# RishWijewardhena/vision-textile-inspection

Hardware: AMD Instinct MI355X
Metric: frames/sec whole-node, YOLOv8n-seg 640x640 bs=64; mask IoU vs CPU ref (higher is better)
Workload: dtype f16x2

## Files before the change

### vision-textile-inspection_amd/csrc/post.hip

```cpp
#include <algorithm>
#include <cmath>
#include <cstdio>
#include <cstring>
#include <type_traits>
#include <vector>

#include "vti_internal.h"

namespace vti {

typedef _Float16 half_t;
typedef _Float16 half8 __attribute__((ext_vector_type(8)));
typedef float f32x4 __attribute__((ext_vector_type(4)));

struct LinTap { int s0, s1, a0, a1; };

__device__ __forceinline__ LinTap lin_tap(int d, int ssize, double scale, bool horizontal) {
    float f = (float)(((double)d + 0.5) * scale - 0.5);
    int s = (int)floorf(f);
    f -= (float)s;
    LinTap t;
    if (horizontal) {
        if (s < 0) { s = 0; f = 0.f; }
        if (s >= ssize - 1) { s = ssize - 1; f = 0.f; }
// ... 217 lines not shown
                if (i >= (nc >> 2)) continue;
                if (v[u].x > best) { best = v[u].x; j = 4 * i; }
                if (v[u].y > best) { best = v[u].y; j = 4 * i + 1; }
                if (v[u].z > best) { best = v[u].z; j = 4 * i + 2; }
                if (v[u].w > best) { best = v[u].w; j = 4 * i + 3; }
            }
            for (int i = q + 4 * MAXV; i < (nc >> 2); i += 4) {
                const float4 w = row[i];
                if (w.x > best) { best = w.x; j = 4 * i; }
                if (w.y > best) { best = w.y; j = 4 * i + 1; }
                if (w.z > best) { best = w.z; j = 4 * i + 2; }
                if (w.w > best) { best = w.w; j = 4 * i + 3; }
            }
        }
#pragma unroll
        for (int o = 1; o <= 2; o <<= 1) {
            const float ob = __shfl_xor(best, o);
            const int oj = __shfl_xor(j, o);
            if (ob > best || (ob == best && oj < j)) { best = ob; j = oj; }
        }
        if (q != 0 || a >= A) return;
    } else {
        a = blockIdx.x * 256 + threadIdx.x;
        if (a >= A) return;
        const float* P = pred + ((size_t)b * A + a) * no;
        best = P[4];
        for (int c = 1; c < nc; ++c) {
            const float v = P[4 + c];
            if (v > best) { best = v; j = c; }
        }
    }
    if (best_out) {
        *(float2*)(best_out + ((size_t)b * A + a) * 2) = make_float2(best, (float)(j == 0x7fffffff ? 0 : j));
        return;
    }
    if (best > conf) {
        char* wsb = ws + (size_t)b * L.per_frame;
        const int idx = atomicAdd(&ncand[b], 1);
        ((unsigned long long*)(wsb + L.keys))[idx] = ((unsigned long long)(~__float_as_uint(best)) << 32) | (unsigned)a;
        ((int*)(wsb + L.cls))[a] = j;
    }
}

#ifdef VTI_STAMPS
__device__ unsigned long long g_nms_stamps[4096 * 8];
#define NMS_STAMP(i)                                                                                   \
    do {                                                                                               \
        if (tid == 0 && b < 4096) {                                                                    \
            unsigned long long t_;                                                                     \
            asm volatile("s_memtime %0\n\ts_waitcnt lgkmcnt(0)" : "=s"(t_)::"memory");                 \
            g_nms_stamps[b * 8 + (i)] = t_;                                                            \
        }                                                                                              \
    } while (0)
#else
#define NMS_STAMP(i) do { } while (0)
#endif

template <typename KeyP, typename BoxP, typename FltP, typename IntP>
__device__ __forceinline__ void nms_body(const float* __restrict__ P, int A, int nc, int nm, int n, double iou, int max_det,
                                         int agnostic, float* __restrict__ D, int* __restrict__ counts, int b,
                                         const unsigned long long* __restrict__ g_keys_in, KeyP keys, BoxP boxes, FltP area,
                                         IntP keep, IntP kid, IntP kcls, unsigned char* suppressed,
                                         const int* __restrict__ cls_of) {
    const int tid = threadIdx.x;
    int Pn = 1;
    while (Pn < n) Pn <<= 1;
    for (int i = tid; i < Pn; i += NMS_THREADS) keys[i] = i < n ? g_keys_in[i] : ~0ull;
    __syncthreads();
    for (int k = 2; k <= Pn; k <<= 1) {
        for (int j = k >> 1; j > 0; j >>= 1) {
            for (int i = tid; i < Pn; i += NMS_THREADS) {
                const int ixj = i ^ j;
                if (ixj > i) {
                    const unsigned long long x = keys[i], y = keys[ixj];
                    const bool up = (i & k) == 0;
                    if ((x > y) == up) { keys[i] = y; keys[ixj] = x; }
                }
            }
            __syncthreads();
        }
    }
    NMS_STAMP(1);
    if (n > NMS_MAX_NMS) n = NMS_MAX_NMS;
    for (int i = tid; i < n; i += NMS_THREADS) {
        const int a = (int)(keys[i] & 0xffffffffu);
        const float* Pa = P + (size_t)a * (4 + nc + nm);
        const float cx = Pa[0], cy = Pa[1], w = Pa[2], h = Pa[3];
        const float dw = w / 2.0f, dh = h / 2.0f;
        const float off = agnostic ? 0.0f : (float)cls_of[a] * NMS_MAX_WH;
        f32x4 bx;
        bx[0] = (cx - dw) + off; bx[1] = (cy - dh) + off; bx[2] = (cx + dw) + off; bx[3] = (cy + dh) + off;
        boxes[i] = bx;
        area[i] = (bx[2] - bx[0]) * (bx[3] - bx[1]);
        suppressed[i] = 0;
    }
    __syncthreads();
    NMS_STAMP(2);
    __shared__ unsigned long long s_rows[64];
    __shared__ int s_kept;
    auto iou_gt = [&](const f32x4& bi, float ai, const f32x4& bj, float aj) -> bool {
        const float xx1 = fmaxf(bi[0], bj[0]), yy1 = fmaxf(bi[1], bj[1]);
        const float xx2 = fminf(bi[2], bj[2]), yy2 = fminf(bi[3], bj[3]);
        const float w = fmaxf(0.0f, xx2 - xx1), h = fmaxf(0.0f, yy2 - yy1);
        const float inter = w * h;
        const float ovr = inter / (ai + aj - inter);
        return (double)ovr > iou;
    };
    int kept = 0;
    if (tid == 0) s_kept = 0;
    for (int base = 0; base < n && kept < max_det; base += 64) {
        const int cnt = min(64, n - base);
        if (tid < 64) s_rows[tid] = 0;
        __syncthreads();
        for (int e = tid; e < 64 * 16; e += NMS_THREADS) {
            const int i = e >> 4, jg = (e & 15) * 4;
            if (i >= cnt || jg + 3 <= i) continue;
            const f32x4 bi = boxes[base + i];
            const float ai = area[base + i];
            unsigned long long m = 0;
            f32x4 bj4[4];
            float aj4[4];
#pragma unroll
            for (int k = 0; k < 4; ++k) {
                const int jc = jg + k < cnt ? jg + k : cnt - 1;
                bj4[k] = boxes[base + jc]; aj4[k] = area[base + jc];
            }
#pragma unroll
            for (int k = 0; k < 4; ++k) {
                const int j = jg + k;
                if (j > i && j < cnt && iou_gt(bi, ai, bj4[k], aj4[k])) m |= 1ull << j;
            }
            if (m) atomicOr(&s_rows[i], m);
        }
        __syncthreads();
        if (tid < 64) {
            const bool alive_l = tid < cnt && !suppressed[base + tid];
            unsigned long long alive = __ballot(alive_l);
            int k_ = kept;
            const unsigned long long myrow = s_rows[tid];
            const int row_lo = (int)(unsigned)myrow, row_hi = (int)(unsigned)(myrow >> 32);
            while (alive && k_ < max_det) {
                const int i = __ffsll((long long)alive) - 1;
                if (tid == 0) keep[k_] = base + i;
                ++k_;
                const unsigned long long ri = (unsigned long long)(unsigned)__builtin_amdgcn_readlane(row_lo, i) |
                                              ((unsigned long long)(unsigned)__builtin_amdgcn_readlane(row_hi, i) << 32);
                alive &= ~(ri | (1ull << i));
            }
            if (tid == 0) s_kept = k_;
        }
        __syncthreads();
        const int kept0 = kept;
        kept = s_kept;
        if (kept < max_det) {
            const int nk = kept - kept0;
            const int rest = n - (base + 64);
            int parts = 1;
            while (parts < 8 && rest * parts * 2 <= NMS_THREADS) parts <<= 1;
            const int part = tid & (parts - 1), lane_j = tid / parts, jstep = NMS_THREADS / parts;
            for (int j = base + 64 + lane_j; j < n; j += jstep) {
                if (suppressed[j]) continue;
                const f32x4 bj = boxes[j];
                const float aj = area[j];
                bool sup = false;
                for (int t = 4 * part; t < nk && !sup; t += 4 * parts) {
                    int ii[4];
                    f32x4 bk[4];
                    float ak[4];
#pragma unroll
                    for (int u = 0; u < 4; ++u) ii[u] = keep[kept0 + (t + u < nk ? t + u : nk - 1)];
#pragma unroll
                    for (int u = 0; u < 4; ++u) { bk[u] = boxes[ii[u]]; ak[u] = area[ii[u]]; }
#pragma unroll
                    for (int u = 0; u < 4; ++u) sup = sup | iou_gt(bk[u], ak[u], bj, aj);
                }
                if (sup) suppressed[j] = 1;
            }
        }
        __syncthreads();
    }
    NMS_STAMP(3);
    for (int k = tid; k < kept; k += NMS_THREADS) {
        const int a = (int)(keys[keep[k]] & 0xffffffffu);
        kid[k] = a;
        kcls[k] = cls_of[a];
    }
    __syncthreads();
    const int row = 6 + nm;
    const unsigned row_magic = (unsigned)((0x100000000ull + (unsigned)row - 1) / (unsigned)row);
    const int nel = kept * row, ntot = max_det * row;
    const int no_ = 4 + nc + nm;
    constexpr int OU = 8;
    for (int e0 = tid; e0 < nel; e0 += OU * NMS_THREADS) {
        float x1[OU], x2[OU];
        int fj[OU];
#pragma unroll
        for (int u = 0; u < OU; ++u) {
            const int e = e0 + u * NMS_THREADS;
            const int ec = e < nel ? e : 0;
            const int k = (int)__umulhi((unsigned)ec, row_magic), f = ec - k * row;
            const int a = kid[k], j = kcls[k];
            const int off1 = f < 4 ? (f & 1) : f == 4 ? 4 + j : f == 5 ? 0 : 4 + nc + (f - 6);
            const int off2 = f < 4 ? 2 + (f & 1) : off1;
            const float* Pa = P + (size_t)a * no_;
            x1[u] = Pa[off1]; x2[u] = Pa[off2];
            fj[u] = (f << 16) | j;
        }
#pragma unroll
        for (int u = 0; u < OU; ++u) {
            const int e = e0 + u * NMS_THREADS;
            const int f = fj[u] >> 16, j = fj[u] & 0xffff;
            const float d_ = x2[u] / 2.0f;
            const float v = f < 2 ? x1[u] - d_ : f < 4 ? x1[u] + d_ : f == 5 ? (float)j : x1[u];
            if (e < nel) D[e] = v;
        }
    }
    for (int e = nel + tid; e < ntot; e += NMS_THREADS) D[e] = 0.f;
    __syncthreads();
    NMS_STAMP(4);
    if (tid == 0) counts[b] = kept;
}

__global__ __launch_bounds__(NMS_THREADS) void nms_kernel(const float* __restrict__ pred, int A, int nc, int nm,
                                                          float conf, double iou, int max_det, int agnostic,
                                                          float* __restrict__ dets, int* __restrict__ counts,
                                                          char* ws, NmsWsLayout L, int* __restrict__ ncand,
                                                          const float* __restrict__ best) {
    extern __shared__ __attribute__((aligned(16))) char smem[];
    unsigned long long* lds_keys = (unsigned long long*)smem;
    f32x4* lds_boxes = (f32x4*)(smem + NMS_LDS_KEYS * 8);
    float* lds_area = (float*)(lds_boxes + NMS_LDS_BOX);
    int* lds_keep = (int*)(lds_area + NMS_LDS_BOX);
    unsigned char* suppressed = (unsigned char*)(lds_keep + 3 * NMS_LDS_BOX);

// ... 39 lines not shown
                 lds_keep + NMS_LDS_BOX, lds_keep + 2 * NMS_LDS_BOX, suppressed, cls_of);
    } else {
        int* g_int = (int*)(wsb + L.keep);
        nms_body(P, A, nc, nm, n, iou, max_det, agnostic, D, counts, b, g_keys, (unsigned long long*)(wsb + L.keys2),
                 (f32x4*)(wsb + L.boxes), (float*)(wsb + L.area), g_int, (int*)(wsb + L.kid), (int*)(wsb + L.kcls), suppressed,
                 cls_of);
    }
}

hipError_t launch_anchor_best(const float* pred, int B, int A, int nc, int nm, float* best, hipStream_t st) {
    if (B == 0) return hipSuccess;
    const int apb = (((4 + nc + nm) | nc) & 3) == 0 ? 64 : 256;
    hipLaunchKernelGGL(nms_scan_kernel, dim3((A + apb - 1) / apb, B), dim3(256), 0, st, pred, A, nc, nm, 0.0f, (char*)nullptr, nms_layout(A),
                       (int*)nullptr, best);
    return hipGetLastError();
}

hipError_t launch_nms(const float* pred, const float* best, int B, int A, int nc, int nm, float conf, double iou, int max_det,
                      int agnostic, float* dets, int* counts, void* ws, hipStream_t st) {
    if (B == 0) return hipSuccess;
    const size_t lds = (size_t)NMS_LDS_KEYS * 8 + (size_t)NMS_LDS_BOX * 32 + (((size_t)A + 15) & ~(size_t)15);
    if (lds > 150 * 1024) return hipErrorInvalidValue;
    const NmsWsLayout L = nms_layout(A);
    int* ncand = (int*)((char*)ws + L.per_frame * (size_t)B);
    if (!best) {
        hipError_t e = hipMemsetAsync(ncand, 0, sizeof(int) * (size_t)B, st);
        if (e != hipSuccess) return e;
        const int apb = (((4 + nc + nm) | nc) & 3) == 0 ? 64 : 256;
        hipLaunchKernelGGL(nms_scan_kernel, dim3((A + apb - 1) / apb, B), dim3(256), 0, st, pred, A, nc, nm, conf, (char*)ws, L, ncand, (float*)nullptr);
    }
    const hipError_t e = launch_lds<nms_kernel>(dim3(B), dim3(NMS_THREADS), lds, st, pred, A, nc, nm, conf, iou, max_det, agnostic,
                                                dets, counts, (char*)ws, L, ncand, best);
#ifdef VTI_STAMPS
    {
        (void)hipStreamSynchronize(st);
        static int calls = 0;
        if (++calls == 3) {
            std::vector<unsigned long long> h(4096 * 8);
            std::vector<int> hc(B), hn(B);
            (void)hipMemcpyFromSymbol(h.data(), HIP_SYMBOL(g_nms_stamps), h.size() * 8);
            (void)hipMemcpy(hc.data(), counts, B * 4, hipMemcpyDeviceToHost);
            (void)hipMemcpy(hn.data(), ncand, B * 4, hipMemcpyDeviceToHost);
            const char* nm_[4] = {"sort", "boxes", "greedy", "output"};
            int worst = 0;
            for (int b = 1; b < B; ++b) if (h[b * 8 + 4] - h[b * 8] > h[worst * 8 + 4] - h[worst * 8]) worst = b;
            fprintf(stderr, "[nms stamps] slowest frame %d: candidates %d kept %d\n", worst, hn[worst], hc[worst]);
            for (int i = 0; i < 4; ++i) {
                std::vector<long long> d;
                for (int b = 0; b < B; ++b) if (hn[b] > 0) d.push_back((long long)(h[b * 8 + i + 1] - h[b * 8 + i]));
                std::sort(d.begin(), d.end());
                fprintf(stderr, "[nms stamps] %-7s median %8lld  max %8lld  slowest-frame %8lld cycles\n", nm_[i],
                        d.empty() ? 0 : d[d.size() / 2], d.empty() ? 0 : d.back(), (long long)(h[worst * 8 + i + 1] - h[worst * 8 + i]));
            }
        }
    }
#endif
    return e;
}

constexpr int MT = 64;
constexpr int ML = MT / 4 + 3;

__global__ __launch_bounds__(256) void mask_offsets_kernel(const int* __restrict__ counts, int B, int max_det,
                                                           int* __restrict__ offsets, int* __restrict__ nitems) {
    extern __shared__ int s_off[];
    for (int b = threadIdx.x; b < B; b += 256) {
        int c = counts[b];
        s_off[b + 1] = c < 0 ? 0 : (c > max_det ? max_det : c);
    }
    if (threadIdx.x == 0) { s_off[0] = 0; *nitems = 0; }
    __syncthreads();
    if (threadIdx.x == 0)
        for (int b = 0; b < B; ++b) s_off[b + 1] += s_off[b];
    __syncthreads();
    for (int b = threadIdx.x; b <= B; b += 256) offsets[b] = s_off[b];
}

__device__ __forceinline__ void mask_slot_owner(const int* __restrict__ offsets, int B, int slot, int& b, int& inst) {
    int lo = 0, hi = B;
    while (hi - lo > 1) { const int mid = (lo + hi) >> 1; if (offsets[mid] <= slot) lo = mid; else hi = mid; }
    b = lo; inst = slot - offsets[lo];
}
__device__ __forceinline__ bool mask_tile_rect(const float* __restrict__ d, int H, int W, int& tx0, int& tx1, int& ty0, int& ty1) {
    const int tiles_x = (W + MT - 1) / MT, tiles_y = (H + MT - 1) / MT;
    const float x1 = d[0] - 8.f, y1 = d[1] - 8.f, x2 = d[2] + 8.f, y2 = d[3] + 8.f;
    tx0 = (int)floorf(x1 / MT); tx1 = (int)floorf(x2 / MT); ty0 = (int)floorf(y1 / MT); ty1 = (int)floorf(y2 / MT);
    tx0 = max(tx0, 0); ty0 = max(ty0, 0); tx1 = min(tx1, tiles_x - 1); ty1 = min(ty1, tiles_y - 1);
    return tx1 >= tx0 && ty1 >= ty0;
}

template <bool FUSED_OFFSETS>
__global__ __launch_bounds__(256) void mask_clear_kernel(const int* __restrict__ counts, int* __restrict__ offsets, int* __restrict__ nitems,
                                                         int B, int max_det, int slot_bytes, int capacity, uint8_t* __restrict__ masks) {
    const int slot = blockIdx.x;
    int total;
    if constexpr (FUSED_OFFSETS) {
        __shared__ int s_c[1025];
        __shared__ int s_tot;
        if (threadIdx.x == 0) s_tot = 0;
        __syncthreads();
        int part = 0;
        for (int b = threadIdx.x; b < B; b += 256) {
            const int c = counts[b], cc = c < 0 ? 0 : (c > max_det ? max_det : c);
            part += cc;
            if (slot == 0) s_c[b + 1] = cc;
        }
        for (int o = 32; o > 0; o >>= 1) part += __shfl_xor(part, o);
        if ((threadIdx.x & 63) == 0) atomicAdd(&s_tot, part);
        __syncthreads();
        total = s_tot;
        if (slot == 0) {
            if (threadIdx.x == 0) {
                s_c[0] = 0; *nitems = 0;
                for (int b = 0; b < B; ++b) s_c[b + 1] += s_c[b];
            }
            __syncthreads();
            for (int b = threadIdx.x; b <= B; b += 256) offsets[b] = s_c[b];
        }
    } else {
        total = offsets[B];
    }
    if (slot >= min(total, capacity)) return;
    uint4* b4 = (uint4*)(masks + (size_t)slot * slot_bytes);
    const int nvec = slot_bytes >> 4;
    for (int v = threadIdx.x; v < nvec; v += 256) b4[v] = make_uint4(0u, 0u, 0u, 0u);
}

__global__ __launch_bounds__(256) void mask_plan_kernel(const float* __restrict__ dets, const int* __restrict__ offsets, int B,
                                                        int max_det, int row, int H, int W, int capacity,
                                                        int2* __restrict__ items, int* __restrict__ nitems) {
    const int slot = blockIdx.x * 256 + threadIdx.x;
    const int total = min(offsets[B], capacity);
    if (slot >= total) return;
    int lo, inst;
    mask_slot_owner(offsets, B, slot, lo, inst);
    const float* d = dets + ((size_t)lo * max_det + inst) * row;
    int tx0, tx1, ty0, ty1;
    if (!mask_tile_rect(d, H, W, tx0, tx1, ty0, ty1)) return;
    const int cnt = (tx1 - tx0 + 1) * (ty1 - ty0 + 1);
    int base = atomicAdd(nitems, cnt);
    for (int ty = ty0; ty <= ty1; ++ty)
        for (int tx = tx0; tx <= tx1; ++tx) items[base++] = make_int2((slot << 12) | (ty << 6) | tx, (int)(((unsigned)lo << 16) | (unsigned)inst));
}

template <bool BYTES>
__device__ __forceinline__ void mask_rows16(const float* lw, const int (&ro)[6], int c0, int c1, float lx1, bool top, float thr,
                                            unsigned& lo, unsigned& hi, uint8_t* __restrict__ out_bytes, int W, int H, int yw, int xg) {
    float hb[6];
#pragma unroll
    for (int j = 0; j < 6; ++j) {
        const float a = lw[ro[j] + c0], b = lw[ro[j] + c1];
        hb[j] = __builtin_fmaf(b - a, lx1, a);
    }
    unsigned l_ = 0u, h_ = 0u;
    constexpr float FR[4] = {0.125f, 0.375f, 0.625f, 0.875f};
#pragma unroll
    for (int r0 = 0; r0 < 16; r0 += 8) {
        unsigned ml[8], mh[8];
#pragma unroll
        for (int q = 0; q < 8; ++q) {
            const int r = r0 + q, j = (r + 2) >> 2;
            float w1 = FR[(r + 2) & 3];
            if (r < 2 && top) w1 = 0.0f;
            const float v = __builtin_fmaf(hb[j + 1] - hb[j], w1, hb[j]);
            if constexpr (BYTES) {
                if (xg < W && yw + r < H) out_bytes[(size_t)(yw + r) * W + xg] = v > thr ? (uint8_t)1 : (uint8_t)0;
            } else {
                const unsigned long long m = __builtin_amdgcn_ballot_w64(v > thr);
                ml[q] = (unsigned)m; mh[q] = (unsigned)(m >> 32);
            }
        }
        if constexpr (!BYTES) {
            if (r0 == 0)
                asm("s_nop 4\n\tv_writelane_b32 %0, %2, 0\n\tv_writelane_b32 %1, %3, 0\n\tv_writelane_b32 %0, %4, 1\n\tv_writelane_b32 %1, %5, 1\n\t"
                    "v_writelane_b32 %0, %6, 2\n\tv_writelane_b32 %1, %7, 2\n\tv_writelane_b32 %0, %8, 3\n\tv_writelane_b32 %1, %9, 3\n\t"
                    "v_writelane_b32 %0, %10, 4\n\tv_writelane_b32 %1, %11, 4\n\tv_writelane_b32 %0, %12, 5\n\tv_writelane_b32 %1, %13, 5\n\t"
                    "v_writelane_b32 %0, %14, 6\n\tv_writelane_b32 %1, %15, 6\n\tv_writelane_b32 %0, %16, 7\n\tv_writelane_b32 %1, %17, 7"
                    : "+v"(l_), "+v"(h_)
// ... 149 lines not shown
    lo = w[0]; hi = w[1];
}

#ifdef VTI_STAMPS
__device__ unsigned long long g_mask_acc[8];
#define MASK_T(i) do { unsigned long long t_; asm volatile("s_memtime %0\n\ts_waitcnt lgkmcnt(0)" : "=s"(t_)::"memory"); \
                       macc[i] += t_ - mprev; mprev = t_; } while (0)
#else
#define MASK_T(i) do { } while (0)
#endif

constexpr int MG = 16;
constexpr int MPTS = ML * ML;
constexpr int MTILES = (MPTS + 15) / 16;
constexpr int MJ = (MTILES + 3) / 4;
constexpr int MROUND = 64;

template <bool F16>
__device__ __forceinline__ float mask_coef_operands(const float (&cf)[32], uint4* dst) {
    float scale = 1.0f;
    if constexpr (F16) {
        float mx = 0.f;
#pragma unroll
        for (int k = 0; k < 32; ++k) mx = fmaxf(mx, fabsf(cf[k]));
        float inv = 1.0f;
        if (!(mx < 3.0e4f)) {
            const int e = (int)((__builtin_bit_cast(unsigned, mx) >> 23) & 255u) - 127 - 13;
            const int ec = e < -100 ? -100 : (e > 100 ? 100 : e);
            scale = __builtin_bit_cast(float, (unsigned)(ec + 127) << 23);
            inv = __builtin_bit_cast(float, (unsigned)(127 - ec) << 23);
        }
#pragma unroll
        for (int q = 0; q < 4; ++q) {
            half8 hh, hl;
#pragma unroll
            for (int k = 0; k < 8; ++k) {
                const float c = cf[8 * q + k] * inv;
                const half_t h = (half_t)c;
                hh[k] = h;
                hl[k] = (half_t)(c - (float)h);
            }
            dst[q] = __builtin_bit_cast(uint4, hh);
            dst[4 + q] = __builtin_bit_cast(uint4, hl);
        }
    } else {
#pragma unroll
        for (int q = 0; q < 8; ++q)
            dst[q] = __builtin_bit_cast(uint4, (f32x4){cf[4 * q], cf[4 * q + 1], cf[4 * q + 2], cf[4 * q + 3]});
    }
    return scale;
}

template <typename T>
__global__ __launch_bounds__(256, sizeof(T) == 2 ? 4 : 3) void masks_group_kernel(const float* __restrict__ dets, const int* __restrict__ offsets,
                                                          const T* __restrict__ proto, int B, int max_det, int Hp, int Wp,
                                                          int H, int W, int mode, int packing, uint8_t* __restrict__ masks,
                                                          int capacity) {
    constexpr bool F16 = sizeof(T) == 2;
    constexpr int ROW = 6 + 32;
    typedef typename std::conditional<F16, half8, f32x4>::type opv;
    constexpr int NOP = F16 ? 1 : 2;
    __shared__ uint4 s_co[MROUND][8];
    __shared__ float4 s_box[MROUND];
    __shared__ float s_scale[MROUND];
    __shared__ unsigned short s_list[MROUND];
    __shared__ int s_n;
    __shared__ float low[MG][ML][MLP];
    const int tid = threadIdx.x, ln = tid & 63, wv = tid >> 6;
    const int li = ln & 15, lg = ln >> 4;
    const int tiles_x = (W + MT - 1) / MT, tiles_y = (H + MT - 1) / MT, tiles = tiles_x * tiles_y;
    const int n = B * tiles;
    const int nx = (int)gridDim.x >> 3, xcd = (int)blockIdx.x & 7, jx = (int)blockIdx.x >> 3;
    const int per = (n + 7) >> 3;
    const int it1 = min(n, (xcd + 1) * per);
    const float wr = (float)((double)Wp / (double)W), hr = (float)((double)Hp / (double)H);
    const float sh = (float)Hp / (float)H, sw = (float)Wp / (float)W;
    const float thr = mode == VTI_MASK_SIGMOID ? 0.5f : 0.0f;
    int prc[MJ];
#pragma unroll
    for (int j = 0; j < MJ; ++j) {
        const int m = wv + 4 * j, pt = 16 * m + li;
        const bool live = m < MTILES && pt < MPTS;
        const int r = live ? pt / ML : ML - 1, c = live ? pt - r * ML : ML;
        prc[j] = (r << 5) | c;
    }
#ifdef VTI_STAMPS
    unsigned long long macc[6] = {0, 0, 0, 0, 0, 0}, mprev, mitems = 0, mpairs = 0;
    asm volatile("s_memtime %0\n\ts_waitcnt lgkmcnt(0)" : "=s"(mprev)::"memory");
#endif
    for (int it = xcd * per + jx; it < it1; it += nx) {
        const int b = it / tiles, t = it - b * tiles;
        const int ty = t / tiles_x, tx = t - ty * tiles_x;
        const int y0 = ty * MT, x0 = tx * MT;
        const int off_b = offsets[b];
        const int n_b = min(offsets[b + 1], capacity) - off_b;
        if (n_b <= 0) continue;
        float fy0 = sh * ((float)y0 + 0.5f) - 0.5f; fy0 = fy0 < 0.f ? 0.f : fy0;
        float fx0 = sw * ((float)x0 + 0.5f) - 0.5f; fx0 = fx0 < 0.f ? 0.f : fx0;
        const int ly0 = (int)fy0, lx0 = (int)fx0;
        opv pb[MJ][NOP];
#pragma unroll
        for (int j = 0; j < MJ; ++j) {
            int q = prc[j];
            asm volatile("" : "+v"(q));
            const int py = ly0 + (q >> 5), px = lx0 + (q & 31);
            const int pyc = py < Hp ? py : Hp - 1, pxc = px < Wp ? px : Wp - 1;
            const T* pp = proto + ((size_t)(b * Hp + pyc) * Wp + pxc) * 32;
            if constexpr (F16) pb[j][0] = *(const half8*)(pp + 8 * lg);
            else { pb[j][0] = *(const f32x4*)(pp + 4 * lg); pb[j][1] = *(const f32x4*)(pp + 16 + 4 * lg); }
        }
        MASK_T(0);
        const int wvy = __builtin_amdgcn_readfirstlane(y0 + 16 * wv);
        const int xg = x0 + ln;
        int kc0 = xg >= 2 ? (xg - 2) >> 2 : 0;
        kc0 = kc0 < Wp - 1 ? kc0 : Wp - 1;
        const int kc1 = kc0 + (kc0 < Wp - 1 ? 1 : 0) - lx0;
        kc0 -= lx0;
        const float lx1 = xg >= 2 ? 0.125f + 0.25f * (float)((xg - 2) & 3) : 0.0f;
        const int rbase = (wvy >> 2) - 1;
        int ro[6];
#pragma unroll
        for (int j = 0; j < 6; ++j) {
            int rr = rbase + j;
            rr = rr < 0 ? 0 : (rr > Hp - 1 ? Hp - 1 : rr);
            ro[j] = (rr - ly0) * MLP;
        }
        const int valid = W - x0;
        const unsigned long long cmask = valid >= 64 ? ~0ull : ((1ull << valid) - 1ull);
        const int yr = y0 + ln;
        const int lrow_off = ((yr >= 2 ? (yr - 2) >> 2 : 0) - ly0) * MLP + (tx > 0 ? 0 : -1);
        const float wy = yr >= 2 ? 0.125f + 0.25f * (float)((yr - 2) & 3) : 0.0f;
        for (int i0 = 0; i0 < n_b; i0 += MROUND) {
            __syncthreads();
            if (wv == 0) {
                const int i = i0 + ln;
                const float* d = dets + ((size_t)b * max_det + (i < n_b ? i : n_b - 1)) * ROW;
                float2 raw[ROW / 2];
#pragma unroll
                for (int k = 0; k < ROW / 2; ++k) raw[k] = *(const float2*)(d + 2 * k);
                const float dd[4] = {raw[0].x, raw[0].y, raw[1].x, raw[1].y};
                int tx0, tx1, ty0, ty1;
                const bool hit = i < n_b && mask_tile_rect(dd, H, W, tx0, tx1, ty0, ty1) && tx >= tx0 && tx <= tx1 && ty >= ty0 && ty <= ty1;
                const unsigned long long bal = __builtin_amdgcn_ballot_w64(hit);
                if (ln == 0) s_n = __builtin_popcountll(bal);
                if (hit) {
                    const int pos = __builtin_amdgcn_mbcnt_hi((unsigned)(bal >> 32), __builtin_amdgcn_mbcnt_lo((unsigned)bal, 0u));
                    s_list[pos] = (unsigned short)ln;
                    s_box[pos] = make_float4(dd[0] * wr, dd[1] * hr, dd[2] * wr, dd[3] * hr);
                    float cf[32];
#pragma unroll
                    for (int k = 0; k < 16; ++k) { cf[2 * k] = raw[3 + k].x; cf[2 * k + 1] = raw[3 + k].y; }
                    s_scale[pos] = mask_coef_operands<F16>(cf, s_co[pos]);
                }
            }
            __syncthreads();
            const int nlist = s_n;
            MASK_T(1);
#ifdef VTI_STAMPS
            ++mitems; mpairs += nlist;
#endif
            for (int g0 = 0; g0 < nlist; g0 += MG) {
                const int ng = min(MG, nlist - g0);
                opv ca[2];
                ca[0] = __builtin_bit_cast(opv, s_co[g0 + li][lg]);
                ca[1] = __builtin_bit_cast(opv, s_co[g0 + li][4 + lg]);
                float4 rb[4];
                float rs[4];
#pragma unroll
                for (int r = 0; r < 4; ++r) {
                    const int u = 4 * lg + r;
                    rb[r] = s_box[g0 + u];
                    rs[r] = s_scale[g0 + u];
                }
#pragma unroll
                for (int j = 0; j < MJ; ++j) {
                    f32x4 acc = (f32x4){0.f, 0.f, 0.f, 0.f};
                    if constexpr (F16) {
                        acc = __builtin_amdgcn_mfma_f32_16x16x32_f16(ca[0], pb[j][0], acc, 0, 0, 0);
                        acc = __builtin_amdgcn_mfma_f32_16x16x32_f16(ca[1], pb[j][0], acc, 0, 0, 0);
                    } else {
#pragma unroll
                        for (int q = 0; q < 2; ++q)
#pragma unroll
                            for (int k = 0; k < 4; ++k) acc = __builtin_amdgcn_mfma_f32_16x16x4f32(ca[q][k], pb[j][q][k], acc, 0, 0, 0);
                    }
                    float v[4];
#pragma unroll
                    for (int r = 0; r < 4; ++r) v[r] = F16 ? acc[r] * rs[r] : acc[r];
                    if (mode == VTI_MASK_SIGMOID) {
#pragma unroll
                        for (int r = 0; r < 4; ++r) v[r] = 1.0f / (1.0f + expf(-v[r]));
                    }
                    int q = prc[j];
                    asm volatile("" : "+v"(q));
                    const int pr = q >> 5, pc = q & 31, py = min(ly0 + pr, Hp - 1), px = min(lx0 + pc, Wp - 1);
                    const float pfc = (float)px, pfr = (float)py;
                    const int pla = pr * MLP + pc;
#pragma unroll
                    for (int r = 0; r < 4; ++r) {
                        const bool inb = pfc >= rb[r].x && pfc < rb[r].z && pfr >= rb[r].y && pfr < rb[r].w;
                        (&low[4 * lg + r][0][0])[pla] = (inb && v[r] == v[r]) ? v[r] : 0.f;
                    }
                }
                MASK_T(2);
                __syncthreads();
                MASK_T(3);
                if (packing != VTI_PACK_U8) {
                    for (int u = wv; u < ng; u += 4) {
                        const int slot = off_b + i0 + (int)s_list[g0 + u];
                        unsigned lo, hi;
                        mask_tile_rows64(&low[u][0][0] + lrow_off, wy, tx == 0, thr, lo, hi);
                        lo &= (unsigned)cmask; hi &= (unsigned)(cmask >> 32);
                        if (yr < H) {
                            unsigned* o = (unsigned*)(masks + ((size_t)slot * H + yr) * (W >> 3) + (x0 >> 3));
                            if (valid >= 64 && !(W & 63)) *(uint2*)o = make_uint2(lo, hi);
                            else {
                                o[0] = lo;
                                if (valid >= 64) o[1] = hi;
                            }
                        }
                    }
                } else if (wvy < H) {
                    for (int u = 0; u < ng; ++u) {
                        const int slot = off_b + i0 + (int)s_list[g0 + u];
                        unsigned lo = 0u, hi = 0u;
                        mask_rows16<true>(&low[u][0][0], ro, kc0, kc1, lx1, wvy == 0, thr, lo, hi, masks + (size_t)slot * H * W, W, H, wvy, xg);
                    }
                }
                MASK_T(4);
                if (g0 + MG < nlist) __syncthreads();
                MASK_T(5);
            }
        }
    }
#ifdef VTI_STAMPS
    if (tid == 0) {
        for (int i = 0; i < 6; ++i) atomicAdd(&g_mask_acc[i], macc[i]);
        atomicAdd(&g_mask_acc[6], mitems); atomicAdd(&g_mask_acc[7], mpairs);
    }
#endif
}

size_t masks_workspace_bytes(int capacity, int H, int W) {
    const size_t tiles = (size_t)((H + MT - 1) / MT) * ((W + MT - 1) / MT);
    return 256 + ((((size_t)capacity * tiles * 8) + 255) & ~(size_t)255);
}

hipError_t launch_masks(int dtype, const float* dets, const int* counts, const void* proto, int B, int max_det, int nm,
                        int Hp, int Wp, int H, int W, int mode, int packing, uint8_t* masks, int capacity,
                        int* offsets, void* ws, hipStream_t st, int wgs_per_cu) {
    if (B == 0) return hipSuccess;
    if (Hp * 4 != H || Wp * 4 != W || nm > 64) return hipErrorInvalidValue;
    int* nitems = (int*)ws;
    int2* items = (int2*)((char*)ws + 256);
    if (max_det > 65535 || B > 32767 || H > 64 * MT || W > 64 * MT || capacity > (1 << 19)) return hipErrorInvalidValue;
    const size_t slot_bytes = (size_t)H * (packing == VTI_PACK_U8 ? W : W / 8);
    if (capacity > 0 && ((slot_bytes & 15) || ((uintptr_t)masks & 15))) return hipErrorInvalidValue;
    if (capacity > 0 && B <= 1024) {
        hipLaunchKernelGGL(mask_clear_kernel<true>, dim3(capacity), dim3(256), 0, st, counts, offsets, nitems, B, max_det, (int)slot_bytes, capacity, masks);
    } else {
        hipLaunchKernelGGL(mask_offsets_kernel, dim3(1), dim3(256), (size_t)(B + 1) * sizeof(int), st, counts, B, max_det, offsets, nitems);
        if (capacity <= 0) return hipGetLastError();
        hipLaunchKernelGGL(mask_clear_kernel<false>, dim3(capacity), dim3(256), 0, st, counts, offsets, nitems, B, max_det, (int)slot_bytes, capacity, masks);
    }
    const int per_cu = dtype == VTI_F16 ? (nm == 32 ? resident_per_cu<masks_group_kernel<half_t>>(256, 4, 8) : resident_per_cu<masks_kernel<half_t>>(256, 4, 8))
                                        : (nm == 32 ? resident_per_cu<masks_group_kernel<float>>(256, 4, 8) : resident_per_cu<masks_kernel<float>>(256, 4, 8));
    int grid = 256 * per_cu;
    if (wgs_per_cu) grid = 256 * std::max(1, std::min(per_cu, wgs_per_cu));
    if (nm == 32) {
        if (dtype == VTI_F16)
            hipLaunchKernelGGL(masks_group_kernel<half_t>, dim3(grid), dim3(256), 0, st, dets, offsets, (const half_t*)proto, B, max_det, Hp, Wp,
                               H, W, mode, packing, masks, capacity);
        else
            hipLaunchKernelGGL(masks_group_kernel<float>, dim3(grid), dim3(256), 0, st, dets, offsets, (const float*)proto, B, max_det, Hp, Wp,
                               H, W, mode, packing, masks, capacity);
#ifdef VTI_STAMPS
        {
            (void)hipStreamSynchronize(st);
            static int calls = 0;
            if (++calls == 3) {
                unsigned long long h[8];
                (void)hipMemcpyFromSymbol(h, HIP_SYMBOL(g_mask_acc), sizeof h);
                const char* nm_[6] = {"decode + issue protos", "list build", "coeffs + MFMA + low", "barrier", "upsample + store", "barrier (next group)"};
                fprintf(stderr, "[mask stamps] %llu (frame, tile) items, %llu (instance, tile) pairs over %d calls (wave 0 of each block; s_memtime ticks per item)\n", h[6], h[7], calls);
                for (int i = 0; i < 6; ++i) fprintf(stderr, "[mask stamps] %-22s %9.1f\n", nm_[i], (double)h[i] / (double)h[6]);
            }
        }
#endif
        return hipGetLastError();
    }
    hipLaunchKernelGGL(mask_plan_kernel, dim3((capacity + 255) / 256), dim3(256), 0, st, dets, offsets, B, max_det, 6 + nm, H, W,
                       capacity, items, nitems);
    if (dtype == VTI_F16)
        hipLaunchKernelGGL(masks_kernel<half_t>, dim3(grid), dim3(256), 0, st, dets, offsets, (const half_t*)proto, B, max_det, nm, Hp, Wp,
                           H, W, mode, packing, masks, items, nitems);
    else
        hipLaunchKernelGGL(masks_kernel<float>, dim3(grid), dim3(256), 0, st, dets, offsets, (const float*)proto, B, max_det, nm, Hp, Wp,
                           H, W, mode, packing, masks, items, nitems);
    return hipGetLastError();
}

__host__ __device__ static inline int native_mask_layout_hd(int Hp, int Wp, int H0, int W0, int packing, int out[6]) {
    if (Hp < 1 || Wp < 1 || H0 < 1 || W0 < 1 || (packing != VTI_PACK_U8 && packing != VTI_PACK_BITS)) return -1;
    const double mh = Hp, mw = Wp;
    const double gh = mh / H0, gw = mw / W0;
    const double gain = gh < gw ? gh : gw;
    const double pad_w = (mw - W0 * gain) / 2, pad_h = (mh - H0 * gain) / 2;
    const int top = (int)pad_h, left = (int)pad_w, bottom = (int)(mh - pad_h), right = (int)(mw - pad_w);
    if (top < 0 || left < 0 || bottom <= top || right <= left || bottom > Hp || right > Wp) return -1;
    const long long row_bytes = packing == VTI_PACK_BITS ? 8LL * ((W0 + 63) / 64) : (long long)W0;
    const long long slot_bytes = row_bytes * H0;
    if (slot_bytes > 0x7fffffffLL) return -1;
    out[0] = top; out[1] = bottom; out[2] = left; out[3] = right; out[4] = (int)row_bytes; out[5] = (int)slot_bytes;
    return 0;
}
int native_mask_layout(int Hp, int Wp, int H0, int W0, int packing, int out[6]) { return native_mask_layout_hd(Hp, Wp, H0, W0, packing, out); }

constexpr int NTW = 64;
constexpr int NPTS = 512;
constexpr int NJ = NPTS / 16 / 4;

struct NativeMaskParams {
    const float* dets;
    const float* xyxy;
    const int* offsets;
    const void* proto;
    uint8_t* masks;
    size_t slot_bytes;
    int B, max_det, Hp, Wp, H0, W0;
    int top, left, inH, inW;
    float sy, sx;
    int th;
    int row_contig, col_contig;
    int mode, packing, row_bytes, capacity;
    const struct NativeFrame* nf;
    const int* tile_prefix;
};

// ... 516 lines not shown
```

Before: 16540.

## Precompute per-instance mask records in clear kernel instead of per-tile decode

The mask-clear kernel, which runs one block per detection slot, now also decodes each detection's tile rectangle, scaled box, and packed coefficient operands into global workspace records. The grouped mask kernel then builds its per-tile instance list with a ballot over those precomputed rectangles and reads coefficients and boxes from global memory. This removes the repeated per-tile decode of the same detection rows and the shared-memory list staging plus two barriers per round. The price is extra workspace, global reads in the inner loop, and a different barrier placement. The change also adds NMS per-phase timing stamps that compile only under VTI_STAMPS.

```diff
diff --git a/vision-textile-inspection_amd/csrc/post.hip b/vision-textile-inspection_amd/csrc/post.hip
--- a/vision-textile-inspection_amd/csrc/post.hip
+++ b/vision-textile-inspection_amd/csrc/post.hip
@@ -293,8 +293,17 @@
             g_nms_stamps[b * 8 + (i)] = t_;                                                            \
         }                                                                                              \
     } while (0)
+#define NMS_TICK(acc)                                                                                  \
+    do {                                                                                               \
+        if (tid == 0) {                                                                                \
+            unsigned long long t_;                                                                     \
+            asm volatile("s_memtime %0\n\ts_waitcnt lgkmcnt(0)" : "=s"(t_)::"memory");                 \
+            acc += t_ - nms_prev; nms_prev = t_;                                                       \
+        }                                                                                              \
+    } while (0)
 #else
 #define NMS_STAMP(i) do { } while (0)
+#define NMS_TICK(acc) do { } while (0)
 #endif
 
 template <typename KeyP, typename BoxP, typename FltP, typename IntP>
@@ -349,10 +358,16 @@
     };
     int kept = 0;
     if (tid == 0) s_kept = 0;
+#ifdef VTI_STAMPS
+    unsigned long long nms_prev = 0, nms_acc[4] = {0, 0, 0, 0};
+    NMS_TICK(nms_acc[0]);
+    nms_acc[0] = 0;
+#endif
     for (int base = 0; base < n && kept < max_det; base += 64) {
         const int cnt = min(64, n - base);
         if (tid < 64) s_rows[tid] = 0;
         __syncthreads();
+        NMS_TICK(nms_acc[0]);
         for (int e = tid; e < 64 * 16; e += NMS_THREADS) {
             const int i = e >> 4, jg = (e & 15) * 4;
             if (i >= cnt || jg + 3 <= i) continue;
@@ -374,6 +389,7 @@
             if (m) atomicOr(&s_rows[i], m);
         }
         __syncthreads();
+        NMS_TICK(nms_acc[1]);
         if (tid < 64) {
             const bool alive_l = tid < cnt && !suppressed[base + tid];
             unsigned long long alive = __ballot(alive_l);
@@ -391,6 +407,7 @@
             if (tid == 0) s_kept = k_;
         }
         __syncthreads();
+        NMS_TICK(nms_acc[2]);
         const int kept0 = kept;
         kept = s_kept;
         if (kept < max_det) {
@@ -419,8 +436,14 @@
             }
         }
         __syncthreads();
+        NMS_TICK(nms_acc[3]);
     }
     NMS_STAMP(3);
+#ifdef VTI_STAMPS
+    if (tid == 0 && b < 4096) {
+        g_nms_stamps[b * 8 + 5] = nms_acc[1]; g_nms_stamps[b * 8 + 6] = nms_acc[2]; g_nms_stamps[b * 8 + 7] = nms_acc[3];
+    }
+#endif
     for (int k = tid; k < kept; k += NMS_THREADS) {
         const int a = (int)(keys[keep[k]] & 0xffffffffu);
         kid[k] = a;
@@ -566,6 +589,8 @@
                 fprintf(stderr, "[nms stamps] %-7s median %8lld  max %8lld  slowest-frame %8lld cycles\n", nm_[i],
                         d.empty() ? 0 : d[d.size() / 2], d.empty() ? 0 : d.back(), (long long)(h[worst * 8 + i + 1] - h[worst * 8 + i]));
             }
+            fprintf(stderr, "[nms stamps] greedy rounds of the slowest frame: A (64 x 64 matrix) %llu  B (walk) %llu  C (later candidates) %llu cycles\n",
+                    h[worst * 8 + 5], h[worst * 8 + 6], h[worst * 8 + 7]);
         }
     }
 #endif
@@ -574,6 +599,24 @@
 
 constexpr int MT = 64;
 constexpr int ML = MT / 4 + 3;
+
+struct MaskRecords { unsigned* rect; float4* box; float* scale; uint4* coef; };
+constexpr unsigned MASK_RECT_EMPTY = 0xffu;
+static inline size_t mask_align16(size_t n) { return (n + 15) & ~(size_t)15; }
+static inline size_t mask_records_bytes(int capacity) {
+    return mask_align16((size_t)capacity * 4) * 2 + (size_t)capacity * (16 + 128);
+}
+static inline MaskRecords mask_records(void* ws, int capacity) {
+    char* p = (char*)ws + 256;
+    MaskRecords r;
+    r.box = (float4*)p; p += (size_t)capacity * 16;
+    r.coef = (uint4*)p; p += (size_t)capacity * 128;
+    r.rect = (unsigned*)p; p += mask_align16((size_t)capacity * 4);
+    r.scale = (float*)p;
+    return r;
+}
+template <bool F16>
+__device__ __forceinline__ float mask_coef_operands(const float (&cf)[32], uint4* dst);
 
 __global__ __launch_bounds__(256) void mask_offsets_kernel(const int* __restrict__ counts, int B, int max_det,
                                                            int* __restrict__ offsets, int* __restrict__ nitems) {
@@ -603,11 +646,14 @@
     return tx1 >= tx0 && ty1 >= ty0;
 }
 
-template <bool FUSED_OFFSETS>
+template <bool FUSED_OFFSETS, int REC>
 __global__ __launch_bounds__(256) void mask_clear_kernel(const int* __restrict__ counts, int* __restrict__ offsets, int* __restrict__ nitems,
-                                                         int B, int max_det, int slot_bytes, int capacity, uint8_t* __restrict__ masks) {
+                                                         int B, int max_det, int slot_bytes, int capacity, uint8_t* __restrict__ masks,
+                                                         const float* __restrict__ dets, int H, int W, MaskRecords rec) {
     const int slot = blockIdx.x;
+    const int ln = threadIdx.x & 63;
     int total;
+    int own_b = 0, own_i = 0;
     if constexpr (FUSED_OFFSETS) {
         __shared__ int s_c[1025];
         __shared__ int s_tot;
@@ -617,27 +663,68 @@
         for (int b = threadIdx.x; b < B; b += 256) {
             const int c = counts[b], cc = c < 0 ? 0 : (c > max_det ? max_det : c);
             part += cc;
-            if (slot == 0) s_c[b + 1] = cc;
+            if (REC || slot == 0) s_c[b + 1] = cc;
         }
         for (int o = 32; o > 0; o >>= 1) part += __shfl_xor(part, o);
         if ((threadIdx.x & 63) == 0) atomicAdd(&s_tot, part);
         __syncthreads();
         total = s_tot;
-        if (slot == 0) {
-            if (threadIdx.x == 0) {
-                s_c[0] = 0; *nitems = 0;
-                for (int b = 0; b < B; ++b) s_c[b + 1] += s_c[b];
-            }
-            __syncthreads();
-            for (int b = threadIdx.x; b <= B; b += 256) offsets[b] = s_c[b];
+        if (slot == 0 && threadIdx.x == 0) {
+            int run = 0;
+            offsets[0] = 0; *nitems = 0;
+            for (int b = 0; b < B; ++b) { run += s_c[b + 1]; offsets[b + 1] = run; }
+        }
+        if (slot >= min(total, capacity)) return;
+        if (REC && threadIdx.x < 64) {
+            const int chunk = (B + 63) >> 6;
+            int sum = 0;
+            for (int k = 0; k < chunk; ++k) { const int b = ln * chunk + k; sum += b < B ? s_c[b + 1] : 0; }
+            int inc = sum;
+#pragma unroll
+            for (int o = 1; o < 64; o <<= 1) { const int t = __shfl_up(inc, o); if (ln >= o) inc += t; }
+            const bool mine = slot >= inc - sum && slot < inc;
+            int fb = 0, fi = 0;
+            if (mine) {
+                int r = slot - (inc - sum);
+                for (int k = 0; k < chunk; ++k) {
+                    const int b = ln * chunk + k, c = b < B ? s_c[b + 1] : 0;
+                    if (r < c) { fb = b; fi = r; break; }
+                    r -= c;
+                }
+            }
+            const int src = __ffsll((long long)__builtin_amdgcn_ballot_w64(mine)) - 1;
+            own_b = __shfl(fb, src); own_i = __shfl(fi, src);
         }
     } else {
         total = offsets[B];
-    }
-    if (slot >= min(total, capacity)) return;
+        if (slot >= min(total, capacity)) return;
+        if (REC && threadIdx.x < 64) mask_slot_owner(offsets, B, slot, own_b, own_i);
+    }
+    constexpr int ROW = 6 + 32;
+    float mine = 0.f;
+    if (REC && threadIdx.x < 64) mine = dets[((size_t)own_b * max_det + own_i) * ROW + (ln < ROW ? ln : ROW - 1)];
     uint4* b4 = (uint4*)(masks + (size_t)slot * slot_bytes);
     const int nvec = slot_bytes >> 4;
     for (int v = threadIdx.x; v < nvec; v += 256) b4[v] = make_uint4(0u, 0u, 0u, 0u);
+    if (REC && threadIdx.x < 64) {
+        float dd[4], cf[32];
+#pragma unroll
+        for (int k = 0; k < 4; ++k) dd[k] = __shfl(mine, k);
+#pragma unroll
+        for (int k = 0; k < 32; ++k) cf[k] = __shfl(mine, 6 + k);
+        uint4 co[8];
+        const float scale = mask_coef_operands<REC == 1>(cf, co);
+        if (ln == 0) {
+            int tx0, tx1, ty0, ty1;
+            const bool any = mask_tile_rect(dd, H, W, tx0, tx1, ty0, ty1);
+            rec.rect[slot] = any ? (unsigned)tx0 | ((unsigned)tx1 << 8) | ((unsigned)ty0 << 16) | ((unsigned)ty1 << 24) : MASK_RECT_EMPTY;
+            const float wr = (float)((double)(W / 4) / (double)W), hr = (float)((double)(H / 4) / (double)H);
+            rec.box[slot] = make_float4(dd[0] * wr, dd[1] * hr, dd[2] * wr, dd[3] * hr);
+            rec.scale[slot] = scale;
+#pragma unroll
+            for (int q = 0; q < 8; ++q) rec.coef[(size_t)slot * 8 + q] = co[q];
+        }
+    }
 }
 
 __global__ __launch_bounds__(256) void mask_plan_kernel(const float* __restrict__ dets, const int* __restrict__ offsets, int B,
@@ -893,20 +980,14 @@
 }
 
 template <typename T>
-__global__ __launch_bounds__(256, sizeof(T) == 2 ? 4 : 3) void masks_group_kernel(const float* __restrict__ dets, const int* __restrict__ offsets,
-                                                          const T* __restrict__ proto, int B, int max_det, int Hp, int Wp,
-                                                          int H, int W, int mode, int packing, uint8_t* __restrict__ masks,
-                                                          int capacity) {
+__global__ __launch_bounds__(256, sizeof(T) == 2 ? 4 : 3) void masks_group_kernel(const int* __restrict__ offsets, const T* __restrict__ proto, int B, int Hp, int Wp,
+                                                             int H, int W, int mode, int packing, uint8_t* __restrict__ masks,
+                                                             int capacity, MaskRecords rec) {
     constexpr bool F16 = sizeof(T) == 2;
-    constexpr int ROW = 6 + 32;
     typedef typename std::conditional<F16, half8, f32x4>::type opv;
     constexpr int NOP = F16 ? 1 : 2;
-    __shared__ uint4 s_co[MROUND][8];
-    __shared__ float4 s_box[MROUND];
-    __shared__ float s_scale[MROUND];
-    __shared__ unsigned short s_list[MROUND];
-    __shared__ int s_n;
-    __shared__ float low[MG][ML][MLP];
+    __shared__ struct { float pad[4]; float low[MG][ML][MLP]; } s_low;
+    float (&low)[MG][ML][MLP] = s_low.low;
     const int tid = threadIdx.x, ln = tid & 63, wv = tid >> 6;
     const int li = ln & 15, lg = ln >> 4;
     const int tiles_x = (W + MT - 1) / MT, tiles_y = (H + MT - 1) / MT, tiles = tiles_x * tiles_y;
@@ -914,8 +995,8 @@
     const int nx = (int)gridDim.x >> 3, xcd = (int)blockIdx.x & 7, jx = (int)blockIdx.x >> 3;
     const int per = (n + 7) >> 3;
     const int it1 = min(n, (xcd + 1) * per);
-    const float wr = (float)((double)Wp / (double)W), hr = (float)((double)Hp / (double)H);
-    const float sh = (float)Hp / (float)H, sw = (float)Wp / (float)W;
+    auto uniform_f = [](float v) { return __builtin_bit_cast(float, __builtin_amdgcn_readfirstlane(__builtin_bit_cast(int, v))); };
+    const float sh = uniform_f((float)Hp / (float)H), sw = uniform_f((float)Wp / (float)W);
     const float thr = mode == VTI_MASK_SIGMOID ? 0.5f : 0.0f;
     int prc[MJ];
 #pragma unroll
@@ -938,7 +1019,7 @@
         if (n_b <= 0) continue;
         float fy0 = sh * ((float)y0 + 0.5f) - 0.5f; fy0 = fy0 < 0.f ? 0.f : fy0;
         float fx0 = sw * ((float)x0 + 0.5f) - 0.5f; fx0 = fx0 < 0.f ? 0.f : fx0;
-        const int ly0 = (int)fy0, lx0 = (int)fx0;
+        const int ly0 = __builtin_amdgcn_readfirstlane((int)fy0), lx0 = __builtin_amdgcn_readfirstlane((int)fx0);
         opv pb[MJ][NOP];
 #pragma unroll
         for (int j = 0; j < MJ; ++j) {
@@ -952,67 +1033,41 @@
         }
         MASK_T(0);
         const int wvy = __builtin_amdgcn_readfirstlane(y0 + 16 * wv);
-        const int xg = x0 + ln;
-        int kc0 = xg >= 2 ? (xg - 2) >> 2 : 0;
-        kc0 = kc0 < Wp - 1 ? kc0 : Wp - 1;
-        const int kc1 = kc0 + (kc0 < Wp - 1 ? 1 : 0) - lx0;
-        kc0 -= lx0;
-        const float lx1 = xg >= 2 ? 0.125f + 0.25f * (float)((xg - 2) & 3) : 0.0f;
-        const int rbase = (wvy >> 2) - 1;
-        int ro[6];
-#pragma unroll
-        for (int j = 0; j < 6; ++j) {
-            int rr = rbase + j;
-            rr = rr < 0 ? 0 : (rr > Hp - 1 ? Hp - 1 : rr);
-            ro[j] = (rr - ly0) * MLP;
-        }
         const int valid = W - x0;
         const unsigned long long cmask = valid >= 64 ? ~0ull : ((1ull << valid) - 1ull);
         const int yr = y0 + ln;
         const int lrow_off = ((yr >= 2 ? (yr - 2) >> 2 : 0) - ly0) * MLP + (tx > 0 ? 0 : -1);
         const float wy = yr >= 2 ? 0.125f + 0.25f * (float)((yr - 2) & 3) : 0.0f;
         for (int i0 = 0; i0 < n_b; i0 += MROUND) {
-            __syncthreads();
-            if (wv == 0) {
-                const int i = i0 + ln;
-                const float* d = dets + ((size_t)b * max_det + (i < n_b ? i : n_b - 1)) * ROW;
-                float2 raw[ROW / 2];
-#pragma unroll
-                for (int k = 0; k < ROW / 2; ++k) raw[k] = *(const float2*)(d + 2 * k);
-                const float dd[4] = {raw[0].x, raw[0].y, raw[1].x, raw[1].y};
-                int tx0, tx1, ty0, ty1;
-                const bool hit = i < n_b && mask_tile_rect(dd, H, W, tx0, tx1, ty0, ty1) && tx >= tx0 && tx <= tx1 && ty >= ty0 && ty <= ty1;
-                const unsigned long long bal = __builtin_amdgcn_ballot_w64(hit);
-                if (ln == 0) s_n = __builtin_popcountll(bal);
-                if (hit) {
-                    const int pos = __builtin_amdgcn_mbcnt_hi((unsigned)(bal >> 32), __builtin_amdgcn_mbcnt_lo((unsigned)bal, 0u));
-                    s_list[pos] = (unsigned short)ln;
-                    s_box[pos] = make_float4(dd[0] * wr, dd[1] * hr, dd[2] * wr, dd[3] * hr);
-                    float cf[32];
-#pragma unroll
-                    for (int k = 0; k < 16; ++k) { cf[2 * k] = raw[3 + k].x; cf[2 * k + 1] = raw[3 + k].y; }
-                    s_scale[pos] = mask_coef_operands<F16>(cf, s_co[pos]);
-                }
-            }
-            __syncthreads();
-            const int nlist = s_n;
+            const int i = i0 + ln;
+            const unsigned rw = rec.rect[off_b + (i < n_b ? i : n_b - 1)];
+            const int rx0 = (int)(rw & 255u), rx1 = (int)((rw >> 8) & 255u), ry0 = (int)((rw >> 16) & 255u), ry1 = (int)(rw >> 24);
+            const bool hit = i < n_b && tx >= rx0 && tx <= rx1 && ty >= ry0 && ty <= ry1;
+            const unsigned long long bal = __builtin_amdgcn_ballot_w64(hit);
+            const int nlist = __builtin_popcountll(bal);
             MASK_T(1);
 #ifdef VTI_STAMPS
             ++mitems; mpairs += nlist;
 #endif
+            if (nlist == 0) continue;
+            const int below = (int)__builtin_amdgcn_mbcnt_hi((unsigned)(bal >> 32), __builtin_amdgcn_mbcnt_lo((unsigned)bal, 0u));
+            const int lidx = __builtin_amdgcn_ds_permute((hit ? below : nlist + ln - below) << 2, ln);
+            const int slot0 = off_b + i0;
             for (int g0 = 0; g0 < nlist; g0 += MG) {
                 const int ng = min(MG, nlist - g0);
+                const uint4* rco = rec.coef + (size_t)(slot0 + __shfl(lidx, min(g0 + li, nlist - 1))) * 8;
                 opv ca[2];
-                ca[0] = __builtin_bit_cast(opv, s_co[g0 + li][lg]);
-                ca[1] = __builtin_bit_cast(opv, s_co[g0 + li][4 + lg]);
+                ca[0] = __builtin_bit_cast(opv, rco[lg]);
+                ca[1] = __builtin_bit_cast(opv, rco[4 + lg]);
                 float4 rb[4];
                 float rs[4];
 #pragma unroll
                 for (int r = 0; r < 4; ++r) {
-                    const int u = 4 * lg + r;
-                    rb[r] = s_box[g0 + u];
-                    rs[r] = s_scale[g0 + u];
+                    const int su = slot0 + __shfl(lidx, min(g0 + 4 * lg + r, nlist - 1));
+                    rb[r] = rec.box[su];
+                    rs[r] = F16 ? rec.scale[su] : 1.0f;
                 }
+                __syncthreads();
 #pragma unroll
                 for (int j = 0; j < MJ; ++j) {
                     f32x4 acc = (f32x4){0.f, 0.f, 0.f, 0.f};
@@ -1048,7 +1103,7 @@
                 MASK_T(3);
                 if (packing != VTI_PACK_U8) {
                     for (int u = wv; u < ng; u += 4) {
-                        const int slot = off_b + i0 + (int)s_list[g0 + u];
+                        const int slot = slot0 + __builtin_amdgcn_readlane(lidx, __builtin_amdgcn_readfirstlane(g0 + u));
                         unsigned lo, hi;
                         mask_tile_rows64(&low[u][0][0] + lrow_off, wy, tx == 0, thr, lo, hi);
                         lo &= (unsigned)cmask; hi &= (unsigned)(cmask >> 32);
@@ -1062,15 +1117,28 @@
                         }
                     }
                 } else if (wvy < H) {
+                    int xg = x0 + ln;
+                    asm volatile("" : "+v"(xg));
+                    int kc0 = xg >= 2 ? (xg - 2) >> 2 : 0;
+                    kc0 = kc0 < Wp - 1 ? kc0 : Wp - 1;
+                    const int kc1 = kc0 + (kc0 < Wp - 1 ? 1 : 0) - lx0;
+                    kc0 -= lx0;
+                    const float lx1 = xg >= 2 ? 0.125f + 0.25f * (float)((xg - 2) & 3) : 0.0f;
+                    const int rbase = (wvy >> 2) - 1;
+                    int ro[6];
+#pragma unroll
+                    for (int j = 0; j < 6; ++j) {
+                        int rr = rbase + j;
+                        rr = rr < 0 ? 0 : (rr > Hp - 1 ? Hp - 1 : rr);
+                        ro[j] = (rr - ly0) * MLP;
+                    }
                     for (int u = 0; u < ng; ++u) {
-                        const int slot = off_b + i0 + (int)s_list[g0 + u];
+                        const int slot = slot0 + __builtin_amdgcn_readlane(lidx, __builtin_amdgcn_readfirstlane(g0 + u));
                         unsigned lo = 0u, hi = 0u;
                         mask_rows16<true>(&low[u][0][0], ro, kc0, kc1, lx1, wvy == 0, thr, lo, hi, masks + (size_t)slot * H * W, W, H, wvy, xg);
                     }
                 }
                 MASK_T(4);
-                if (g0 + MG < nlist) __syncthreads();
-                MASK_T(5);
             }
         }
     }
@@ -1084,7 +1152,16 @@
 
 size_t masks_workspace_bytes(int capacity, int H, int W) {
     const size_t tiles = (size_t)((H + MT - 1) / MT) * ((W + MT - 1) / MT);
-    return 256 + ((((size_t)capacity * tiles * 8) + 255) & ~(size_t)255);
+    return 256 + ((std::max((size_t)capacity * tiles * 8, mask_records_bytes(capacity)) + 255) & ~(size_t)255);
+}
+
+template <bool FUSED_OFFSETS>
+static void launch_mask_clear(int rec_kind, const int* counts, int* offsets, int* nitems, int B, int max_det, int slot_bytes, int capacity,
+                              uint8_t* masks, const float* dets, int H, int W, const MaskRecords& rec, hipStream_t st) {
+    const dim3 grid(capacity), block(256);
+    if (rec_kind == 1) hipLaunchKernelGGL((mask_clear_kernel<FUSED_OFFSETS, 1>), grid, block, 0, st, counts, offsets, nitems, B, max_det, slot_bytes, capacity, masks, dets, H, W, rec);
+    else if (rec_kind == 2) hipLaunchKernelGGL((mask_clear_kernel<FUSED_OFFSETS, 2>), grid, block, 0, st, counts, offsets, nitems, B, max_det, slot_bytes, capacity, masks, dets, H, W, rec);
+    else hipLaunchKernelGGL((mask_clear_kernel<FUSED_OFFSETS, 0>), grid, block, 0, st, counts, offsets, nitems, B, max_det, slot_bytes, capacity, masks, dets, H, W, rec);
 }
 
 hipError_t launch_masks(int dtype, const float* dets, const int* counts, const void* proto, int B, int max_det, int nm,
@@ -1096,13 +1173,15 @@
     int2* items = (int2*)((char*)ws + 256);
     if (max_det > 65535 || B > 32767 || H > 64 * MT || W > 64 * MT || capacity > (1 << 19)) return hipErrorInvalidValue;
     const size_t slot_bytes = (size_t)H * (packing == VTI_PACK_U8 ? W : W / 8);
-    if (capacity > 0 && ((slot_bytes & 15) || ((uintptr_t)masks & 15))) return hipErrorInvalidValue;
+    if (capacity > 0 && ((slot_bytes & 15) || ((uintptr_t)masks & 15) || ((uintptr_t)ws & 15))) return hipErrorInvalidValue;
+    const int rec_kind = nm == 32 ? (dtype == VTI_F16 ? 1 : 2) : 0;
+    const MaskRecords rec = mask_records(ws, std::max(capacity, 0));
     if (capacity > 0 && B <= 1024) {
-        hipLaunchKernelGGL(mask_clear_kernel<true>, dim3(capacity), dim3(256), 0, st, counts, offsets, nitems, B, max_det, (int)slot_bytes, capacity, masks);
+        launch_mask_clear<true>(rec_kind, counts, offsets, nitems, B, max_det, (int)slot_bytes, capacity, masks, dets, H, W, rec, st);
     } else {
         hipLaunchKernelGGL(mask_offsets_kernel, dim3(1), dim3(256), (size_t)(B + 1) * sizeof(int), st, counts, B, max_det, offsets, nitems);
         if (capacity <= 0) return hipGetLastError();
-        hipLaunchKernelGGL(mask_clear_kernel<false>, dim3(capacity), dim3(256), 0, st, counts, offsets, nitems, B, max_det, (int)slot_bytes, capacity, masks);
+        launch_mask_clear<false>(rec_kind, counts, offsets, nitems, B, max_det, (int)slot_bytes, capacity, masks, dets, H, W, rec, st);
     }
     const int per_cu = dtype == VTI_F16 ? (nm == 32 ? resident_per_cu<masks_group_kernel<half_t>>(256, 4, 8) : resident_per_cu<masks_kernel<half_t>>(256, 4, 8))
                                         : (nm == 32 ? resident_per_cu<masks_group_kernel<float>>(256, 4, 8) : resident_per_cu<masks_kernel<float>>(256, 4, 8));
@@ -1110,11 +1189,11 @@
     if (wgs_per_cu) grid = 256 * std::max(1, std::min(per_cu, wgs_per_cu));
     if (nm == 32) {
         if (dtype == VTI_F16)
-            hipLaunchKernelGGL(masks_group_kernel<half_t>, dim3(grid), dim3(256), 0, st, dets, offsets, (const half_t*)proto, B, max_det, Hp, Wp,
-                               H, W, mode, packing, masks, capacity);
+            hipLaunchKernelGGL(masks_group_kernel<half_t>, dim3(grid), dim3(256), 0, st, offsets, (const half_t*)proto, B, Hp, Wp,
+                               H, W, mode, packing, masks, capacity, rec);
         else
-            hipLaunchKernelGGL(masks_group_kernel<float>, dim3(grid), dim3(256), 0, st, dets, offsets, (const float*)proto, B, max_det, Hp, Wp,
-                               H, W, mode, packing, masks, capacity);
+            hipLaunchKernelGGL(masks_group_kernel<float>, dim3(grid), dim3(256), 0, st, offsets, (const float*)proto, B, Hp, Wp,
+                               H, W, mode, packing, masks, capacity, rec);
 #ifdef VTI_STAMPS
         {
             (void)hipStreamSynchronize(st);
@@ -1122,9 +1201,9 @@
             if (++calls == 3) {
                 unsigned long long h[8];
                 (void)hipMemcpyFromSymbol(h, HIP_SYMBOL(g_mask_acc), sizeof h);
-                const char* nm_[6] = {"decode + issue protos", "list build", "coeffs + MFMA + low", "barrier", "upsample + store", "barrier (next group)"};
+                const char* nm_[5] = {"decode + issue protos", "list build", "records + MFMA + low", "barrier", "upsample + store"};
                 fprintf(stderr, "[mask stamps] %llu (frame, tile) items, %llu (instance, tile) pairs over %d calls (wave 0 of each block; s_memtime ticks per item)\n", h[6], h[7], calls);
-                for (int i = 0; i < 6; ++i) fprintf(stderr, "[mask stamps] %-22s %9.1f\n", nm_[i], (double)h[i] / (double)h[6]);
+                for (int i = 0; i < 5; ++i) fprintf(stderr, "[mask stamps] %-22s %9.1f\n", nm_[i], (double)h[i] / (double)h[6]);
             }
         }
 #endif
```

After: 16570 (median of 2 runs). No clear change (+0.2%).
